# aymenboudhina/Multimodal_VQVAE_compression_audio_tactile

Hardware: AMD Instinct MI355X
Metric: encode+VQ+decode token-frames/sec (1 frame = 13.33 ms of paired 24 kHz audio+tactile) (higher is better)
Workload: dtype f32

## Files before the change

multimodal_vqvae_compression_audio_tactile_amd/csrc/api.hip:

```cpp
#include <hip/hip_runtime.h>
#include <stdarg.h>
#include <math.h>
#include <stdio.h>
#include <string.h>
#include "../../include/mvq.h"
#include "conv_dispatch.hpp"
#include "kernels_small.hpp"

#include <map>
#include <string>
#include <vector>

namespace mvq {
namespace {
struct ProfRec { std::string name; double flops; hipEvent_t e0, e1; };
std::vector<ProfRec> g_prof;
std::vector<hipEvent_t> g_prof_pool;
bool g_prof_on = false;
hipError_t g_prof_err = hipSuccess;
hipEvent_t prof_event()
{
    if (!g_prof_pool.empty()) { hipEvent_t e = g_prof_pool.back(); g_prof_pool.pop_back(); return e; }
    hipEvent_t e = nullptr;
    const hipError_t rc = hipEventCreate(&e);
    if (rc != hipSuccess) { if (g_prof_err == hipSuccess) g_prof_err = rc; return nullptr; }
    return e;
}
}
bool prof_enabled() { return g_prof_on; }
int prof_begin(const char* kernel_name, double flops, hipStream_t s)
{
    if (!g_prof_on) return -1;
    ProfRec r{kernel_name, flops, prof_event(), nullptr};
    if (!r.e0) return -1;
    r.e1 = prof_event();
    if (!r.e1) { g_prof_pool.push_back(r.e0); return -1; }
    const hipError_t rc = hipEventRecord(r.e0, s);
    if (rc != hipSuccess) {
        if (g_prof_err == hipSuccess) g_prof_err = rc;
        g_prof_pool.push_back(r.e0); g_prof_pool.push_back(r.e1);
        return -1;
    }
    g_prof.push_back(r);
    return (int)g_prof.size() - 1;
}
void prof_end(int idx, hipStream_t s)
{
    if (idx < 0 || idx >= (int)g_prof.size()) return;
    const hipError_t rc = hipEventRecord(g_prof[idx].e1, s);
    if (rc != hipSuccess && g_prof_err == hipSuccess) g_prof_err = rc;
}
}

namespace {
thread_local char g_err[512] = "";

int fail(int code, const char* fmt, ...)
{
    va_list ap; va_start(ap, fmt); vsnprintf(g_err, sizeof(g_err), fmt, ap); va_end(ap);
    return code;
}
int hipfail(hipError_t e, const char* what)
{
    return fail(MVQ_EHIP, "%s: %s", what, hipGetErrorString(e));
}
inline hipStream_t S(void* s) { return reinterpret_cast<hipStream_t>(s); }
}
namespace mvq {
void set_last_error(const char* msg) { snprintf(g_err, sizeof(g_err), "%s", msg); }
}
namespace {
inline int conv_out_len(int tin, int ks, int stride, int dil, int pad)
{
    const int span = tin + 2 * pad - dil * (ks - 1) - 1;
    return span < 0 ? 0 : span / stride + 1;
}
}

extern "C" {

int mvq_profile_begin(void)
{
    for (auto& r : mvq::g_prof) { mvq::g_prof_pool.push_back(r.e0); mvq::g_prof_pool.push_back(r.e1); }
    mvq::g_prof.clear();
    mvq::g_prof_err = hipSuccess;
    mvq::g_prof_on = true;
    return MVQ_OK;
}

// ... 36 lines not shown
    std::map<std::string, mvq_profile_entry> agg;
    for (auto& r : mvq::g_prof) {
        hipError_t e = hipEventSynchronize(r.e1);
        if (e != hipSuccess) { recycle(); return hipfail(e, "profile_end: hipEventSynchronize"); }
        float ms = 0.0f;
        e = hipEventElapsedTime(&ms, r.e0, r.e1);
        if (e != hipSuccess) { recycle(); return hipfail(e, "profile_end: hipEventElapsedTime"); }
        auto it = agg.find(r.name);
        if (it == agg.end()) {
            mvq_profile_entry z{};
            snprintf(z.kernel, sizeof(z.kernel), "%s", r.name.c_str());
            it = agg.emplace(r.name, z).first;
        }
        it->second.seconds += 1e-3 * (double)ms;
        it->second.flops += r.flops;
        it->second.launches += 1;
    }
    recycle();
    int i = 0;
    for (auto& kv : agg) {
        if (i >= max_entries) break;
        out[i++] = kv.second;
    }
    *n_entries = i;
    if (n_total) *n_total = (int)agg.size();
    return MVQ_OK;
}

int mvq_abi_version(void) { return 3; }
unsigned mvq_build_flags(void) { return getenv("MVQ_NO_DMA") ? 0x100u : 0u; }
const char* mvq_last_error(void) { return g_err; }

int mvq_device_query(int* cu_count, int* lds_bytes_per_cu, char* arch, int arch_len)
{
    int dev = 0;
    hipError_t e = hipGetDevice(&dev);
    if (e != hipSuccess) return hipfail(e, "hipGetDevice");
    hipDeviceProp_t p;
    e = hipGetDeviceProperties(&p, dev);
    if (e != hipSuccess) return hipfail(e, "hipGetDeviceProperties");
    if (cu_count) *cu_count = p.multiProcessorCount;
    if (lds_bytes_per_cu) *lds_bytes_per_cu = (int)p.maxSharedMemoryPerMultiProcessor;
    if (arch && arch_len > 0) { strncpy(arch, p.gcnArchName, arch_len - 1); arch[arch_len - 1] = 0; }
    return MVQ_OK;
}

int mvq_weight_norm_f32(const float* v, const float* g, float* w, int rows, int inner, void* stream)
{
    if (!v || !g || !w || rows <= 0 || inner <= 0) return fail(MVQ_EINVAL, "weight_norm: bad argument");
    hipError_t e = mvq::launch_weight_norm(v, g, w, rows, inner, S(stream));
    return e == hipSuccess ? MVQ_OK : hipfail(e, "weight_norm");
}

size_t mvq_conv1d_packed_floats(int cin, int cout, int ks)
{
    if (cin <= 0 || cout <= 0 || ks <= 0) return 0;
    return (size_t)cin * ks * mvq::conv_mpad(cout);
}

int mvq_conv1d_pack_f32(const float* w, float* wp, int cin, int cout, int ks, void* stream)
{
    if (!w || !wp || cin <= 0 || cout <= 0 || ks <= 0) return fail(MVQ_EINVAL, "conv1d_pack: bad argument");
    hipError_t e = mvq::launch_pack_conv1d(w, wp, cin, cout, ks, mvq::conv_mpad(cout), S(stream));
    return e == hipSuccess ? MVQ_OK : hipfail(e, "conv1d_pack");
}

size_t mvq_conv_transpose1d_packed_floats(int cin, int cout, int stride)
{
    if (cin <= 0 || cout <= 0 || stride <= 0) return 0;
    return (size_t)cin * 2 * mvq::conv_mpad(cout * stride);
}

int mvq_conv_transpose1d_pack_f32(const float* w, float* wp, int cin, int cout, int stride, void* stream)
{
    if (!w || !wp || cin <= 0 || cout <= 0 || stride <= 0) return fail(MVQ_EINVAL, "conv_transpose1d_pack: bad argument");
    hipError_t e = mvq::launch_pack_convtr(w, wp, cin, cout, stride, mvq::conv_mpad(cout * stride), S(stream));
    return e == hipSuccess ? MVQ_OK : hipfail(e, "conv_transpose1d_pack");
}

static hipError_t dispatch_conv1d(const mvq::ConvArgs& a, int ks, int stride, int dil, hipStream_t s)
{
    const int bm = mvq::conv_tile_bm(a.Cout);
    hipError_t e = hipErrorInvalidValue;
    if (a.Cout >= 16 && a.Cin >= 32 && mvq::conv_underfilled(a) && mvq::conv_lat_wanted(a, ks)) {
        e = mvq::launch_conv_lat(a, ks, stride, dil, s);
        if (e != hipErrorInvalidValue) return e;
    }
    if (a.Cout >= 32 && a.Cin >= 32) {
        if (ks == 7 && stride == 1 && a.Cin % 8 == 0) e = mvq::launch_conv_k7(a, dil, bm, s);
        else if (ks == 1 && stride == 1 && dil == 1 && a.Cin % 32 == 0) e = mvq::launch_conv_k1k3(a, 1, bm, s);
        else if (ks == 3 && stride == 1 && dil == 1 && a.Cin % 16 == 0) e = mvq::launch_conv_k1k3(a, 3, bm, s);
        else if (ks == 2 * stride && dil == 1 && a.Cin % 16 == 0) e = mvq::launch_conv_strided(a, stride, bm, s);
    }
    return e;
}

static hipError_t dispatch_convtr(const mvq::ConvArgs& a, hipStream_t s)
{
    if (a.Cin % 32 != 0 || a.Mrows < 64) return hipErrorInvalidValue;
    return mvq::launch_conv_tr(a, mvq::conv_tile_bm(a.Mrows), s);
}

size_t mvq_bf16x3_split_bytes(int batch, int c, int t)
{
    if (batch <= 0 || c <= 0 || t <= 0) return 0;
    return (size_t)batch * c * t * 6;
}
int mvq_bf16x3_split_f32(const float* x, void* xs, int batch, int c, int t, void* stream)
{
    if (batch < 0 || c <= 0 || t < 0 || c % 8 != 0) return fail(MVQ_EINVAL, "bf16x3_split: bad shape B=%d C=%d T=%d (C %% 8 == 0)", batch, c, t);
    if (batch == 0 || t == 0) return MVQ_OK;
    if (!x || !xs) return fail(MVQ_EINVAL, "bf16x3_split: null tensor");
    if ((reinterpret_cast<uintptr_t>(xs) & 15) != 0) return fail(MVQ_EINVAL, "bf16x3_split: xs must be 16-byte aligned");
    const hipError_t e = mvq::launch_bf16x3_split(x, xs, batch, c, t, S(stream));
    return e == hipSuccess ? MVQ_OK : hipfail(e, "bf16x3_split");
}
size_t mvq_conv1d_k7_bf16x3_packed_bytes(int cout, int cin)
{
    if (cout <= 0 || cin <= 0 || mvq::bf16x6_tile_rows(cout) == 0 || cin % 16 != 0) return 0;
    return (size_t)cout * cin * 7 * 6;
}
int mvq_conv1d_k7_pack_bf16x3(const float* w, void* wq, int cout, int cin, int dgrad, void* stream)
{
    if (cout <= 0 || cin <= 0 || mvq::bf16x6_tile_rows(cout) == 0 || cin % 16 != 0)
        return fail(MVQ_EINVAL, "conv1d_k7_pack_bf16x3: Cout %d must be a multiple of 128 or 96 and Cin %d of 16", cout, cin);
    if (!w || !wq) return fail(MVQ_EINVAL, "conv1d_k7_pack_bf16x3: null tensor");
    if ((reinterpret_cast<uintptr_t>(wq) & 15) != 0) return fail(MVQ_EINVAL, "conv1d_k7_pack_bf16x3: wq must be 16-byte aligned");
    const hipError_t e = mvq::launch_bf16x3_pack_k7(w, wq, cout, cin, dgrad != 0, S(stream));
    return e == hipSuccess ? MVQ_OK : hipfail(e, "conv1d_k7_pack_bf16x3");
}
int mvq_conv1d_k7_bf16x6_f32(const void* xs, const void* wq, const float* bias, const float* alpha_out, float* y, float* y2,
                             const float* dsn_src, const float* dsn_alpha, const float* residual,
                             int batch, int cin, int t, int cout, int dil, int tvalid, void* stream)
{
    if (batch < 0 || cin <= 0 || cout <= 0 || t < 0 || mvq::bf16x6_tile_rows(cout) == 0 || cin % 16 != 0)
        return fail(MVQ_EINVAL, "conv1d_k7_bf16x6: bad shape B=%d Cin=%d T=%d Cout=%d (Cout %% 128 or 96, Cin %% 16)", batch, cin, t, cout);
    if (dil != 1 && dil != 3 && dil != 9) return fail(MVQ_EINVAL, "conv1d_k7_bf16x6: dilation %d not in {1, 3, 9}", dil);
    if (tvalid < 0 || tvalid > t) return fail(MVQ_EINVAL, "conv1d_k7_bf16x6: tvalid %d outside [0, %d]", tvalid, t);
    if (batch == 0 || t == 0) return MVQ_OK;
    if (!xs || !wq || !y) return fail(MVQ_EINVAL, "conv1d_k7_bf16x6: null tensor");
    if (((reinterpret_cast<uintptr_t>(xs) | reinterpret_cast<uintptr_t>(wq)) & 15) != 0)
        return fail(MVQ_EINVAL, "conv1d_k7_bf16x6: xs / wq must be 16-byte aligned");
    if ((long long)batch * ((t + 127) / 128) > 0x7fffffffLL) return fail(MVQ_EINVAL, "conv1d_k7_bf16x6: grid too large");
    if (y2 && !alpha_out) return fail(MVQ_EINVAL, "conv1d_k7_bf16x6: the dual output needs alpha_out");
    if ((dsn_src != nullptr) != (dsn_alpha != nullptr)) return fail(MVQ_EINVAL, "conv1d_k7_bf16x6: dsn_src and dsn_alpha go together");
    mvq::K7Extra ex; ex.y2 = y2; ex.dsn_src = dsn_src; ex.dsn_alpha = dsn_alpha; ex.residual = residual;
    const hipError_t e = mvq::launch_conv_k7_bf16x6(xs, wq, bias, alpha_out, y, batch, cin, t, cout, dil, tvalid, ex, S(stream));
    return e == hipSuccess ? MVQ_OK : hipfail(e, "conv1d_k7_bf16x6");
}

int mvq_f16x2_split_f32(const float* x, void* xs, uint32_t* xamax, int batch, int c, int t, void* stream)
{
    if (batch < 0 || c <= 0 || t < 0 || c % 8 != 0) return fail(MVQ_EINVAL, "f16x2_split: bad shape B=%d C=%d T=%d (C %% 8 == 0)", batch, c, t);
    if (batch == 0 || t == 0) return MVQ_OK;
    if (!x || !xs || !xamax) return fail(MVQ_EINVAL, "f16x2_split: null tensor");
    if ((reinterpret_cast<uintptr_t>(xs) & 15) != 0) return fail(MVQ_EINVAL, "f16x2_split: xs must be 16-byte aligned");
    const hipError_t e = mvq::launch_f16x2_split(x, xs, xamax, batch, c, t, S(stream));
    return e == hipSuccess ? MVQ_OK : hipfail(e, "f16x2_split");
}
size_t mvq_conv1d_k7_f16x2_packed_bytes(int cout, int cin)
{
    if (cout <= 0 || cin <= 0 || mvq::bf16x6_tile_rows(cout) == 0 || cin % 16 != 0) return 0;
    return (size_t)cout * cin * 7 * 4;
}
int mvq_conv1d_k7_pack_f16x2(const float* w, void* wq, uint32_t* wamax, int cout, int cin, int dgrad, void* stream)
{
    if (cout <= 0 || cin <= 0 || mvq::bf16x6_tile_rows(cout) == 0 || cin % 16 != 0)
// ... 832 lines not shown
```

multimodal_vqvae_compression_audio_tactile_amd/csrc/conv_k1k3.hip:

```cpp
#include "conv_dispatch.hpp"
namespace mvq {
hipError_t launch_conv_k1k3(const ConvArgs& a, int ks, int bm, hipStream_t s)
{
    if (ks == 1) {
        if (bm != 96 && conv_prefer_small_tiles(a)) return launch_conv1d_mfma<1, 1, 1, 32, 1, 1, 2, 2, 0>(a, s);
        if (bm == 128) {
            const int tail = a.name_out ? 0 : conv_tail_width(a);
            if (tail) {
                ConvArgs m = a, t = a;
                m.n_tiles_max = a.Ncols / 128;
                t.n_base = m.n_tiles_max * 128;
                hipError_t e = launch_conv1d_mfma<1, 1, 1, 16, 2, 2, 2, 2, 0>(m, s);
                if (e != hipSuccess) return e;
                return tail == 96 ? launch_conv1d_mfma<1, 1, 1, 16, 1, 3, 4, 1, 0>(t, s)
                                  : launch_conv1d_mfma<1, 1, 1, 16, 2, 1, 2, 2, 0>(t, s);
            }
        }
        switch (bm) {
            case 128: return launch_conv1d_mfma<1, 1, 1, 16, 2, 2, 2, 2, 0>(a, s);
            case 96:
                      return (long)a.B * ((a.Ncols + 127) / 128) * ((a.Mrows + 95) / 96) < 200
                                 ? launch_conv1d_mfma<1, 1, 1, 32, 3, 1, 1, 4, 0>(a, s)
                                 : launch_conv1d_mfma<1, 1, 1, 16, 3, 1, 1, 4, 0>(a, s);
            case 64:  return launch_conv1d_mfma<1, 1, 1, 16, 2, 2, 1, 4, 0>(a, s);
        }
    } else if (ks == 3) {
        if (bm != 96 && conv_prefer_small_tiles(a)) return launch_conv1d_mfma<3, 1, 1, 16, 1, 1, 2, 2, 0>(a, s);
        if (bm == 128 && a.Ncols <= 96) return launch_conv1d_mfma<3, 1, 1, 8, 1, 3, 4, 1, 0>(a, s);
        switch (bm) {
            case 128: return conv_dma_rows_ok(a) ? launch_conv1d_mfma<3, 1, 1, 8, 2, 2, 2, 2, 0>(a, s)
                                                 : launch_conv1d_mfma<3, 1, 1, 16, 2, 2, 2, 2, 0>(a, s);
        }
    }
    return hipErrorInvalidValue;
}
}
```

multimodal_vqvae_compression_audio_tactile_amd/csrc/conv_k7.hip:

```cpp
#include "conv_dispatch.hpp"
namespace mvq {
template <int DIL>
static hipError_t k7(const ConvArgs& a, int bm, hipStream_t s)
{
    if (DIL == 1 && bm == 128 && a.Ncols <= 96 && !conv_prefer_small_tiles(a))
        return launch_conv1d_mfma<7, 1, 1, 4, 1, 3, 4, 1, 0>(a, s);
    if (bm != 96 && conv_prefer_small_tiles(a)) return launch_conv1d_mfma<7, 1, DIL, 8, 1, 1, 2, 2, 0>(a, s);
    if (bm == 128) {
        const int tail = a.name_out ? 0 : conv_tail_width(a);
        if (tail) {
            ConvArgs m = a, t = a;
            m.n_tiles_max = a.Ncols / 128;
            t.n_base = m.n_tiles_max * 128;
            hipError_t e = launch_conv1d_mfma<7, 1, DIL, 4, 2, 2, 2, 2, 0>(m, s);
            if (e != hipSuccess) return e;
            return tail == 96 ? launch_conv1d_mfma<7, 1, DIL, 4, 1, 3, 4, 1, 0>(t, s)
                              : launch_conv1d_mfma<7, 1, DIL, 4, 2, 1, 2, 2, 0>(t, s);
        }
    }
    switch (bm) {
        case 128: return launch_conv1d_mfma<7, 1, DIL, 4, 2, 2, 2, 2, 0>(a, s);
        case 96:  return launch_conv1d_mfma<7, 1, DIL, 4, 3, 1, 1, 4, 0>(a, s);
        case 64:  return launch_conv1d_mfma<7, 1, DIL, 8, 2, 2, 1, 4, 0>(a, s);
    }
    return hipErrorInvalidValue;
}
hipError_t launch_conv_k7(const ConvArgs& a, int dil, int bm, hipStream_t s)
{
    switch (dil) {
        case 1: return k7<1>(a, bm, s);
        case 3: return k7<3>(a, bm, s);
        case 9: return k7<9>(a, bm, s);
    }
    return hipErrorInvalidValue;
}
}
```

multimodal_vqvae_compression_audio_tactile_amd/csrc/conv_strided.hip:

```cpp
#include "conv_dispatch.hpp"
namespace mvq {
hipError_t launch_conv_strided(const ConvArgs& a, int stride, int bm, hipStream_t s)
{
    const bool dma = conv_dma_rows_ok(a);
    if (bm == 96 && stride == 2) return dma ? launch_conv1d_mfma<4, 2, 1, 4, 3, 1, 1, 4, 0>(a, s) : launch_conv1d_mfma<4, 2, 1, 8, 3, 1, 1, 4, 0>(a, s);
    if (bm != 128) return hipErrorInvalidValue;
    if (conv_prefer_small_tiles(a)) {
        switch (stride) {
            case 2: return launch_conv1d_mfma<4, 2, 1, 16, 1, 1, 2, 2, 0>(a, s);
            case 4: return launch_conv1d_mfma<8, 4, 1, 8, 1, 1, 2, 2, 0>(a, s);
            case 5: return launch_conv1d_mfma<10, 5, 1, 4, 1, 1, 2, 2, 0>(a, s);
            case 8: return launch_conv1d_mfma<16, 8, 1, 4, 1, 1, 2, 2, 0>(a, s);
        }
    }
    const int tail = a.name_out ? 0 : conv_tail_width(a);
    if (tail && (stride == 4 || stride == 5)) {
        ConvArgs m = a, t = a;
        m.n_tiles_max = a.Ncols / 128;
        t.n_base = m.n_tiles_max * 128;
        hipError_t e = stride == 4 ? (dma ? launch_conv1d_mfma<8, 4, 1, 2, 2, 2, 2, 2, 0>(m, s) : launch_conv1d_mfma<8, 4, 1, 4, 2, 2, 2, 2, 0>(m, s))
                                   : launch_conv1d_mfma<10, 5, 1, 2, 2, 2, 2, 2, 0>(m, s);
        if (e != hipSuccess) return e;
        if (stride == 4) return tail == 96 ? launch_conv1d_mfma<8, 4, 1, 2, 1, 3, 4, 1, 0>(t, s) : launch_conv1d_mfma<8, 4, 1, 2, 2, 1, 2, 2, 0>(t, s);
        return tail == 96 ? launch_conv1d_mfma<10, 5, 1, 2, 1, 3, 4, 1, 0>(t, s) : launch_conv1d_mfma<10, 5, 1, 2, 2, 1, 2, 2, 0>(t, s);
    }
    switch (stride) {
        case 2: return dma ? launch_conv1d_mfma<4, 2, 1, 4, 2, 2, 2, 2, 0>(a, s) : launch_conv1d_mfma<4, 2, 1, 8, 2, 2, 2, 2, 0>(a, s);
        case 4: return dma ? launch_conv1d_mfma<8, 4, 1, 2, 2, 2, 2, 2, 0>(a, s) : launch_conv1d_mfma<8, 4, 1, 4, 2, 2, 2, 2, 0>(a, s);
        case 5: return launch_conv1d_mfma<10, 5, 1, 2, 2, 2, 2, 2, 0>(a, s);
        case 8: if (a.Ncols <= 96) return dma ? launch_conv1d_mfma<16, 8, 1, 1, 1, 3, 4, 1, 0>(a, s) : launch_conv1d_mfma<16, 8, 1, 2, 1, 3, 4, 1, 0>(a, s);
                return dma ? launch_conv1d_mfma<16, 8, 1, 1, 2, 2, 2, 2, 0>(a, s) : launch_conv1d_mfma<16, 8, 1, 2, 2, 2, 2, 2, 0>(a, s);
    }
    return hipErrorInvalidValue;
}
}
```

multimodal_vqvae_compression_audio_tactile_amd/csrc/conv_tr.hip:

```cpp
#include "conv_dispatch.hpp"
namespace mvq {
hipError_t launch_conv_tr(const ConvArgs& a, int bm, hipStream_t s)
{
    if (bm == 128 && conv_prefer_small_tiles(a)) {
        switch (a.up_s) {
            case 8: return launch_conv1d_mfma<2, 1, 1, 32, 1, 1, 2, 2, 8>(a, s);
            case 5: return launch_conv1d_mfma<2, 1, 1, 32, 1, 1, 2, 2, 5>(a, s);
            case 4: return launch_conv1d_mfma<2, 1, 1, 32, 1, 1, 2, 2, 4>(a, s);
            case 2: return launch_conv1d_mfma<2, 1, 1, 32, 1, 1, 2, 2, 2>(a, s);
        }
    }
    const bool dma = conv_dma_rows_ok(a);
    const int tail = (a.name_out || bm != 128) ? 0 : conv_tail_width(a);
    if (tail && (a.up_s == 4 || a.up_s == 5)) {
        ConvArgs m = a, t = a;
        m.n_tiles_max = a.Ncols / 128;
        t.n_base = m.n_tiles_max * 128;
        hipError_t e;
        if (a.up_s == 4) e = dma ? launch_conv1d_mfma<2, 1, 1, 8, 2, 2, 2, 2, 4>(m, s) : launch_conv1d_mfma<2, 1, 1, 16, 2, 2, 2, 2, 4>(m, s);
        else e = dma ? launch_conv1d_mfma<2, 1, 1, 8, 2, 2, 2, 2, 5>(m, s) : launch_conv1d_mfma<2, 1, 1, 16, 2, 2, 2, 2, 5>(m, s);
        if (e != hipSuccess) return e;
        if (a.up_s == 4) return tail == 96 ? launch_conv1d_mfma<2, 1, 1, 8, 1, 3, 4, 1, 4>(t, s) : launch_conv1d_mfma<2, 1, 1, 8, 2, 1, 2, 2, 4>(t, s);
        return tail == 96 ? launch_conv1d_mfma<2, 1, 1, 8, 1, 3, 4, 1, 5>(t, s) : launch_conv1d_mfma<2, 1, 1, 8, 2, 1, 2, 2, 5>(t, s);
    }
    const bool narrow = bm == 128 && a.Ncols <= 96;
    switch (a.up_s) {
        case 8: if (bm == 128 && narrow) return dma ? launch_conv1d_mfma<2, 1, 1, 8, 1, 3, 4, 1, 8>(a, s) : launch_conv1d_mfma<2, 1, 1, 16, 1, 3, 4, 1, 8>(a, s);
                if (bm == 128) return dma ? launch_conv1d_mfma<2, 1, 1, 8, 2, 2, 2, 2, 8>(a, s) : launch_conv1d_mfma<2, 1, 1, 16, 2, 2, 2, 2, 8>(a, s);
                break;
        case 5: if (bm == 128) return dma ? launch_conv1d_mfma<2, 1, 1, 8, 2, 2, 2, 2, 5>(a, s) : launch_conv1d_mfma<2, 1, 1, 16, 2, 2, 2, 2, 5>(a, s);
                break;
        case 4: if (bm == 128) return dma ? launch_conv1d_mfma<2, 1, 1, 8, 2, 2, 2, 2, 4>(a, s) : launch_conv1d_mfma<2, 1, 1, 16, 2, 2, 2, 2, 4>(a, s);
                break;
        case 2: if (bm == 96) return dma ? launch_conv1d_mfma<2, 1, 1, 8, 3, 1, 1, 4, 2>(a, s) : launch_conv1d_mfma<2, 1, 1, 16, 3, 1, 1, 4, 2>(a, s);
                if (bm == 128) return dma ? launch_conv1d_mfma<2, 1, 1, 8, 2, 2, 2, 2, 2>(a, s) : launch_conv1d_mfma<2, 1, 1, 16, 2, 2, 2, 2, 2>(a, s);
                break;
    }
    return hipErrorInvalidValue;
}
}
```

multimodal_vqvae_compression_audio_tactile_amd/dac.py:

```python
from __future__ import annotations

import math
import os
from typing import List, Optional

import torch
import torch.nn as nn

from . import ops
from ._lib import MvqError

ENC_RATES = (2, 4, 5, 8)
DEC_RATES = (8, 5, 4, 2)

PLAN_ENV = ("MVQ_RU_PRESNAKED", "MVQ_VPACKED_LATENTS", "MVQ_PACKED_MIN_BATCH", "MVQ_PACKED_LATENTS", "MVQ_PY_PLAN")
PLAN_OVERRIDES = {k: os.environ[k] for k in PLAN_ENV if k in os.environ}
HOST_ENV_SEEN = {k: os.environ[k] for k in ("MVQ_TWO_STREAM_MAX_BATCH", "MVQ_AR_FUSED_MAX_BATCH", "MVQ_AR_STAGED_MAX_BATCH") if k in os.environ}
USE_STACKS = not PLAN_OVERRIDES


def plan_overrides():
    return sorted(PLAN_OVERRIDES) + sorted(HOST_ENV_SEEN)


class _Packed:

    def __init__(self):
        self._key = None
        self.value = None

    def invalidate(self):
        self._key = None

    def get(self, params, make):
        key = tuple((id(p), p._version, p.data_ptr(), str(p.device)) for p in params)
        if key != self._key:
            self.value = make()
            self._key = key
        return self.value


def _stack_of(mod, describe):
    st = getattr(mod, "_stack_state", None)
    if st is None or st.get("probe") is None:
        probe = describe()
        named = dict(mod.named_parameters())
        st = mod._stack_state = {"probe": probe, "params": [named[n] for n in probe.param_names()], "stamp": None, "stack": None}
    ps = st["params"]
    stamp = (sum(p._version for p in ps), ps[0].data_ptr(), ps[-1].data_ptr(), ps[0].device)
    if stamp != st["stamp"]:
        st["stack"] = st["probe"].bind(ps)
        st["stamp"] = stamp
    return st["stack"]


class Snake1d(nn.Module):

    def __init__(self, channels: int):
        super().__init__()
        self.alpha = nn.Parameter(torch.ones(1, channels, 1))

    def flat(self) -> torch.Tensor:
        return self.alpha.detach().reshape(-1).float().contiguous()


class _WNKeys:

    def _load_from_state_dict(self, state_dict, prefix, *args, **kwargs):
        for new, old in (("parametrizations.weight.original0", "weight_g"), ("parametrizations.weight.original1", "weight_v")):
            if prefix + new in state_dict and prefix + old not in state_dict:
                state_dict[prefix + old] = state_dict.pop(prefix + new)
        super()._load_from_state_dict(state_dict, prefix, *args, **kwargs)


class WNConv1d(_WNKeys, nn.Module):

    def __init__(self, cin, cout, kernel_size, stride=1, dilation=1, padding=0):
        super().__init__()
        self.cin, self.cout, self.ks = cin, cout, kernel_size
        self.stride, self.dilation, self.padding = stride, dilation, padding
        v = torch.randn(cout, cin, kernel_size) / math.sqrt(cin * kernel_size)
        self.weight_g = nn.Parameter(v.reshape(cout, -1).norm(dim=1).reshape(cout, 1, 1))
        self.weight_v = nn.Parameter(v)
        self.bias = nn.Parameter(torch.zeros(cout))
        self._packed = _Packed()

    def packed(self) -> torch.Tensor:
        return self._packed.get((self.weight_g, self.weight_v),
                                lambda: ops.pack_conv1d(ops.weight_norm(self.weight_v.detach(), self.weight_g.detach())))

    def folded_weight(self) -> torch.Tensor:
        return ops.weight_norm(self.weight_v.detach(), self.weight_g.detach())

    def packed_bf16x3(self) -> torch.Tensor:
        if not hasattr(self, "_packed_bf"):
            self._packed_bf = _Packed()
        return self._packed_bf.get((self.weight_g, self.weight_v), lambda: ops.pack_conv1d_k7_bf16x3(self.folded_weight()))

    def packed_f16x2(self):
        if not hasattr(self, "_packed_f16"):
# ... 520 lines not shown
```

Measured before the change: 60700.

## Add analytic cost model to pick conv MFMA tile shape per launch

Introduces a per-family tile cost model using measured efficiency tables, CU wave quantization and LDS-limited residency. Each conv launcher (k1, k3, k7, strided, transposed) builds candidate tiles and keeps the current choice unless another is predicted cheaper by a margin. An MVQ_CONV_TILE env override is also added for forcing a tile. The aim is to reduce wave-quantization and underfill losses on small grids; the risk is model error picking a slower tile, plus getenv overhead on every launch.

After: 60650 (median of 2 runs). Within noise of the previous version (-0.1%).

```diff
diff --git a/multimodal_vqvae_compression_audio_tactile_amd/csrc/api.hip b/multimodal_vqvae_compression_audio_tactile_amd/csrc/api.hip
--- a/multimodal_vqvae_compression_audio_tactile_amd/csrc/api.hip
+++ b/multimodal_vqvae_compression_audio_tactile_amd/csrc/api.hip
@@ -5,6 +5,7 @@
 #include <string.h>
 #include "../../include/mvq.h"
 #include "conv_dispatch.hpp"
+#include "conv_tile_model.hpp"
 #include "kernels_small.hpp"
 
 #include <map>
@@ -207,7 +208,8 @@
 {
     const int bm = mvq::conv_tile_bm(a.Cout);
     hipError_t e = hipErrorInvalidValue;
-    if (a.Cout >= 16 && a.Cin >= 32 && mvq::conv_underfilled(a) && mvq::conv_lat_wanted(a, ks)) {
+    if (a.Cout >= 16 && a.Cin >= 32 && mvq::conv_underfilled(a) && mvq::conv_lat_wanted(a, ks) &&
+        mvq::conv_tile_forced() == mvq::TILE_NONE) {
         e = mvq::launch_conv_lat(a, ks, stride, dil, s);
         if (e != hipErrorInvalidValue) return e;
     }
diff --git a/multimodal_vqvae_compression_audio_tactile_amd/csrc/conv_k1k3.hip b/multimodal_vqvae_compression_audio_tactile_amd/csrc/conv_k1k3.hip
--- a/multimodal_vqvae_compression_audio_tactile_amd/csrc/conv_k1k3.hip
+++ b/multimodal_vqvae_compression_audio_tactile_amd/csrc/conv_k1k3.hip
@@ -1,10 +1,19 @@
 #include "conv_dispatch.hpp"
+#include "conv_tile_model.hpp"
 namespace mvq {
 hipError_t launch_conv_k1k3(const ConvArgs& a, int ks, int bm, hipStream_t s)
 {
     if (ks == 1) {
-        if (bm != 96 && conv_prefer_small_tiles(a)) return launch_conv1d_mfma<1, 1, 1, 32, 1, 1, 2, 2, 0>(a, s);
         if (bm == 128) {
+            const TileCand c[5] = {tile_cand<1, 1, 1, 16, 2, 2, 2, 2, 0>(TILE_128x128, a), tile_cand<1, 1, 1, 16, 1, 3, 4, 1, 0>(TILE_128x96, a),
+                                   tile_cand<1, 1, 1, 16, 2, 1, 2, 2, 0>(TILE_128x64, a), tile_cand<1, 1, 1, 16, 1, 2, 2, 2, 0>(TILE_64x128, a),
+                                   tile_cand<1, 1, 1, 32, 1, 1, 2, 2, 0>(TILE_64x64, a)};
+            switch (conv_choose_tile(a, FAM_K1, a.Cin, 1, c, 5, conv_prefer_small_tiles(a) ? TILE_64x64 : TILE_128x128)) {
+                case TILE_128x96: return launch_conv1d_mfma<1, 1, 1, 16, 1, 3, 4, 1, 0>(a, s);
+                case TILE_128x64: return launch_conv1d_mfma<1, 1, 1, 16, 2, 1, 2, 2, 0>(a, s);
+                case TILE_64x128: return launch_conv1d_mfma<1, 1, 1, 16, 1, 2, 2, 2, 0>(a, s);
+                case TILE_64x64:  return launch_conv1d_mfma<1, 1, 1, 32, 1, 1, 2, 2, 0>(a, s);
+            }
             const int tail = a.name_out ? 0 : conv_tail_width(a);
             if (tail) {
                 ConvArgs m = a, t = a;
@@ -15,22 +24,32 @@
                 return tail == 96 ? launch_conv1d_mfma<1, 1, 1, 16, 1, 3, 4, 1, 0>(t, s)
                                   : launch_conv1d_mfma<1, 1, 1, 16, 2, 1, 2, 2, 0>(t, s);
             }
+            return launch_conv1d_mfma<1, 1, 1, 16, 2, 2, 2, 2, 0>(a, s);
         }
         switch (bm) {
-            case 128: return launch_conv1d_mfma<1, 1, 1, 16, 2, 2, 2, 2, 0>(a, s);
             case 96:
                       return (long)a.B * ((a.Ncols + 127) / 128) * ((a.Mrows + 95) / 96) < 200
                                  ? launch_conv1d_mfma<1, 1, 1, 32, 3, 1, 1, 4, 0>(a, s)
                                  : launch_conv1d_mfma<1, 1, 1, 16, 3, 1, 1, 4, 0>(a, s);
-            case 64:  return launch_conv1d_mfma<1, 1, 1, 16, 2, 2, 1, 4, 0>(a, s);
+            case 64: {
+                const TileCand c[2] = {tile_cand<1, 1, 1, 16, 2, 2, 1, 4, 0>(TILE_64x256, a), tile_cand<1, 1, 1, 32, 1, 1, 2, 2, 0>(TILE_64x64, a)};
+                return conv_choose_tile(a, FAM_K1, a.Cin, 1, c, 2, conv_prefer_small_tiles(a) ? TILE_64x64 : TILE_64x256) == TILE_64x64
+                           ? launch_conv1d_mfma<1, 1, 1, 32, 1, 1, 2, 2, 0>(a, s) : launch_conv1d_mfma<1, 1, 1, 16, 2, 2, 1, 4, 0>(a, s);
+            }
         }
     } else if (ks == 3) {
-        if (bm != 96 && conv_prefer_small_tiles(a)) return launch_conv1d_mfma<3, 1, 1, 16, 1, 1, 2, 2, 0>(a, s);
-        if (bm == 128 && a.Ncols <= 96) return launch_conv1d_mfma<3, 1, 1, 8, 1, 3, 4, 1, 0>(a, s);
-        switch (bm) {
-            case 128: return conv_dma_rows_ok(a) ? launch_conv1d_mfma<3, 1, 1, 8, 2, 2, 2, 2, 0>(a, s)
-                                                 : launch_conv1d_mfma<3, 1, 1, 16, 2, 2, 2, 2, 0>(a, s);
+        if (bm != 128) {
+            if (bm != 96 && conv_prefer_small_tiles(a)) return launch_conv1d_mfma<3, 1, 1, 16, 1, 1, 2, 2, 0>(a, s);
+            return hipErrorInvalidValue;
         }
+        const bool dma = conv_dma_rows_ok(a);
+        const TileCand c[3] = {dma ? tile_cand<3, 1, 1, 8, 2, 2, 2, 2, 0>(TILE_128x128, a) : tile_cand<3, 1, 1, 16, 2, 2, 2, 2, 0>(TILE_128x128, a),
+                               tile_cand<3, 1, 1, 8, 1, 3, 4, 1, 0>(TILE_128x96, a), tile_cand<3, 1, 1, 16, 1, 1, 2, 2, 0>(TILE_64x64, a)};
+        switch (conv_choose_tile(a, FAM_K3, a.Cin * 3, 3, c, 3, conv_prefer_small_tiles(a) ? TILE_64x64 : (a.Ncols <= 96 ? TILE_128x96 : TILE_128x128))) {
+            case TILE_64x64:  return launch_conv1d_mfma<3, 1, 1, 16, 1, 1, 2, 2, 0>(a, s);
+            case TILE_128x96: return launch_conv1d_mfma<3, 1, 1, 8, 1, 3, 4, 1, 0>(a, s);
+        }
+        return dma ? launch_conv1d_mfma<3, 1, 1, 8, 2, 2, 2, 2, 0>(a, s) : launch_conv1d_mfma<3, 1, 1, 16, 2, 2, 2, 2, 0>(a, s);
     }
     return hipErrorInvalidValue;
 }
diff --git a/multimodal_vqvae_compression_audio_tactile_amd/csrc/conv_k7.hip b/multimodal_vqvae_compression_audio_tactile_amd/csrc/conv_k7.hip
--- a/multimodal_vqvae_compression_audio_tactile_amd/csrc/conv_k7.hip
+++ b/multimodal_vqvae_compression_audio_tactile_amd/csrc/conv_k7.hip
@@ -1,29 +1,37 @@
 #include "conv_dispatch.hpp"
+#include "conv_tile_model.hpp"
 namespace mvq {
 template <int DIL>
 static hipError_t k7(const ConvArgs& a, int bm, hipStream_t s)
 {
-    if (DIL == 1 && bm == 128 && a.Ncols <= 96 && !conv_prefer_small_tiles(a))
-        return launch_conv1d_mfma<7, 1, 1, 4, 1, 3, 4, 1, 0>(a, s);
-    if (bm != 96 && conv_prefer_small_tiles(a)) return launch_conv1d_mfma<7, 1, DIL, 8, 1, 1, 2, 2, 0>(a, s);
-    if (bm == 128) {
-        const int tail = a.name_out ? 0 : conv_tail_width(a);
-        if (tail) {
-            ConvArgs m = a, t = a;
-            m.n_tiles_max = a.Ncols / 128;
-            t.n_base = m.n_tiles_max * 128;
-            hipError_t e = launch_conv1d_mfma<7, 1, DIL, 4, 2, 2, 2, 2, 0>(m, s);
-            if (e != hipSuccess) return e;
-            return tail == 96 ? launch_conv1d_mfma<7, 1, DIL, 4, 1, 3, 4, 1, 0>(t, s)
-                              : launch_conv1d_mfma<7, 1, DIL, 4, 2, 1, 2, 2, 0>(t, s);
-        }
+    if (bm == 96) return launch_conv1d_mfma<7, 1, DIL, 4, 3, 1, 1, 4, 0>(a, s);
+    if (bm == 64) {
+        const TileCand c[2] = {tile_cand<7, 1, DIL, 8, 2, 2, 1, 4, 0>(TILE_64x256, a), tile_cand<7, 1, DIL, 8, 1, 1, 2, 2, 0>(TILE_64x64, a)};
+        const int t = conv_choose_tile(a, DIL == 9 ? FAM_K7D9 : FAM_K7, a.Cin * 7, 7, c, 2, conv_prefer_small_tiles(a) ? TILE_64x64 : TILE_64x256);
+        return t == TILE_64x64 ? launch_conv1d_mfma<7, 1, DIL, 8, 1, 1, 2, 2, 0>(a, s) : launch_conv1d_mfma<7, 1, DIL, 8, 2, 2, 1, 4, 0>(a, s);
     }
-    switch (bm) {
-        case 128: return launch_conv1d_mfma<7, 1, DIL, 4, 2, 2, 2, 2, 0>(a, s);
-        case 96:  return launch_conv1d_mfma<7, 1, DIL, 4, 3, 1, 1, 4, 0>(a, s);
-        case 64:  return launch_conv1d_mfma<7, 1, DIL, 8, 2, 2, 1, 4, 0>(a, s);
+    if (bm != 128) return hipErrorInvalidValue;
+    const int today = conv_prefer_small_tiles(a) ? TILE_64x64 : ((DIL == 1 && a.Ncols <= 96) ? TILE_128x96 : TILE_128x128);
+    const TileCand c[5] = {tile_cand<7, 1, DIL, 4, 2, 2, 2, 2, 0>(TILE_128x128, a), tile_cand<7, 1, DIL, 4, 1, 3, 4, 1, 0>(TILE_128x96, a),
+                           tile_cand<7, 1, DIL, 4, 2, 1, 2, 2, 0>(TILE_128x64, a), tile_cand<7, 1, DIL, 4, 1, 2, 2, 2, 0>(TILE_64x128, a),
+                           tile_cand<7, 1, DIL, 8, 1, 1, 2, 2, 0>(TILE_64x64, a)};
+    switch (conv_choose_tile(a, DIL == 9 ? FAM_K7D9 : FAM_K7, a.Cin * 7, 7, c, 5, today)) {
+        case TILE_128x96: return launch_conv1d_mfma<7, 1, DIL, 4, 1, 3, 4, 1, 0>(a, s);
+        case TILE_128x64: return launch_conv1d_mfma<7, 1, DIL, 4, 2, 1, 2, 2, 0>(a, s);
+        case TILE_64x128: return launch_conv1d_mfma<7, 1, DIL, 4, 1, 2, 2, 2, 0>(a, s);
+        case TILE_64x64:  return launch_conv1d_mfma<7, 1, DIL, 8, 1, 1, 2, 2, 0>(a, s);
     }
-    return hipErrorInvalidValue;
+    const int tail = a.name_out ? 0 : conv_tail_width(a);
+    if (tail) {
+        ConvArgs m = a, t = a;
+        m.n_tiles_max = a.Ncols / 128;
+        t.n_base = m.n_tiles_max * 128;
+        hipError_t e = launch_conv1d_mfma<7, 1, DIL, 4, 2, 2, 2, 2, 0>(m, s);
+        if (e != hipSuccess) return e;
+        return tail == 96 ? launch_conv1d_mfma<7, 1, DIL, 4, 1, 3, 4, 1, 0>(t, s)
+                          : launch_conv1d_mfma<7, 1, DIL, 4, 2, 1, 2, 2, 0>(t, s);
+    }
+    return launch_conv1d_mfma<7, 1, DIL, 4, 2, 2, 2, 2, 0>(a, s);
 }
 hipError_t launch_conv_k7(const ConvArgs& a, int dil, int bm, hipStream_t s)
 {
diff --git a/multimodal_vqvae_compression_audio_tactile_amd/csrc/conv_strided.hip b/multimodal_vqvae_compression_audio_tactile_amd/csrc/conv_strided.hip
--- a/multimodal_vqvae_compression_audio_tactile_amd/csrc/conv_strided.hip
+++ b/multimodal_vqvae_compression_audio_tactile_amd/csrc/conv_strided.hip
@@ -1,16 +1,57 @@
 #include "conv_dispatch.hpp"
+#include "conv_tile_model.hpp"
 namespace mvq {
 hipError_t launch_conv_strided(const ConvArgs& a, int stride, int bm, hipStream_t s)
 {
     const bool dma = conv_dma_rows_ok(a);
     if (bm == 96 && stride == 2) return dma ? launch_conv1d_mfma<4, 2, 1, 4, 3, 1, 1, 4, 0>(a, s) : launch_conv1d_mfma<4, 2, 1, 8, 3, 1, 1, 4, 0>(a, s);
     if (bm != 128) return hipErrorInvalidValue;
-    if (conv_prefer_small_tiles(a)) {
+    {
+        const int ktot = a.Cin * 2 * stride;
+        const int today = conv_prefer_small_tiles(a) ? TILE_64x64 : ((stride == 8 && a.Ncols <= 96) ? TILE_128x96 : TILE_128x128);
+        TileCand c[4];
+        int n = 0;
         switch (stride) {
-            case 2: return launch_conv1d_mfma<4, 2, 1, 16, 1, 1, 2, 2, 0>(a, s);
-            case 4: return launch_conv1d_mfma<8, 4, 1, 8, 1, 1, 2, 2, 0>(a, s);
-            case 5: return launch_conv1d_mfma<10, 5, 1, 4, 1, 1, 2, 2, 0>(a, s);
-            case 8: return launch_conv1d_mfma<16, 8, 1, 4, 1, 1, 2, 2, 0>(a, s);
+            case 2: c[n++] = dma ? tile_cand<4, 2, 1, 4, 2, 2, 2, 2, 0>(TILE_128x128, a) : tile_cand<4, 2, 1, 8, 2, 2, 2, 2, 0>(TILE_128x128, a);
+                    c[n++] = tile_cand<4, 2, 1, 16, 1, 1, 2, 2, 0>(TILE_64x64, a);
+                    break;
+            case 4: c[n++] = dma ? tile_cand<8, 4, 1, 2, 2, 2, 2, 2, 0>(TILE_128x128, a) : tile_cand<8, 4, 1, 4, 2, 2, 2, 2, 0>(TILE_128x128, a);
+                    c[n++] = tile_cand<8, 4, 1, 2, 1, 3, 4, 1, 0>(TILE_128x96, a);
+                    c[n++] = tile_cand<8, 4, 1, 2, 2, 1, 2, 2, 0>(TILE_128x64, a);
+                    c[n++] = tile_cand<8, 4, 1, 8, 1, 1, 2, 2, 0>(TILE_64x64, a);
+                    break;
+            case 5: c[n++] = tile_cand<10, 5, 1, 2, 2, 2, 2, 2, 0>(TILE_128x128, a);
+                    c[n++] = tile_cand<10, 5, 1, 2, 1, 3, 4, 1, 0>(TILE_128x96, a);
+                    c[n++] = tile_cand<10, 5, 1, 2, 2, 1, 2, 2, 0>(TILE_128x64, a);
+                    c[n++] = tile_cand<10, 5, 1, 4, 1, 1, 2, 2, 0>(TILE_64x64, a);
+                    break;
+            case 8: c[n++] = dma ? tile_cand<16, 8, 1, 1, 2, 2, 2, 2, 0>(TILE_128x128, a) : tile_cand<16, 8, 1, 2, 2, 2, 2, 2, 0>(TILE_128x128, a);
+                    c[n++] = dma ? tile_cand<16, 8, 1, 1, 1, 3, 4, 1, 0>(TILE_128x96, a) : tile_cand<16, 8, 1, 2, 1, 3, 4, 1, 0>(TILE_128x96, a);
+                    c[n++] = tile_cand<16, 8, 1, 4, 1, 1, 2, 2, 0>(TILE_64x64, a);
+                    break;
+            default: return hipErrorInvalidValue;
+        }
+        const int t = conv_choose_tile(a, stride == 2 ? FAM_S2 : stride == 4 ? FAM_S4 : stride == 5 ? FAM_S5 : FAM_S8, ktot, 2 * stride, c, n, today);
+        if (t == TILE_64x64) {
+            switch (stride) {
+                case 2: return launch_conv1d_mfma<4, 2, 1, 16, 1, 1, 2, 2, 0>(a, s);
+                case 4: return launch_conv1d_mfma<8, 4, 1, 8, 1, 1, 2, 2, 0>(a, s);
+                case 5: return launch_conv1d_mfma<10, 5, 1, 4, 1, 1, 2, 2, 0>(a, s);
+                case 8: return launch_conv1d_mfma<16, 8, 1, 4, 1, 1, 2, 2, 0>(a, s);
+            }
+        }
+        if (t == TILE_128x96) {
+            switch (stride) {
+                case 4: return launch_conv1d_mfma<8, 4, 1, 2, 1, 3, 4, 1, 0>(a, s);
+                case 5: return launch_conv1d_mfma<10, 5, 1, 2, 1, 3, 4, 1, 0>(a, s);
+                case 8: return dma ? launch_conv1d_mfma<16, 8, 1, 1, 1, 3, 4, 1, 0>(a, s) : launch_conv1d_mfma<16, 8, 1, 2, 1, 3, 4, 1, 0>(a, s);
+            }
+        }
+        if (t == TILE_128x64) {
+            switch (stride) {
+                case 4: return launch_conv1d_mfma<8, 4, 1, 2, 2, 1, 2, 2, 0>(a, s);
+                case 5: return launch_conv1d_mfma<10, 5, 1, 2, 2, 1, 2, 2, 0>(a, s);
+            }
         }
     }
     const int tail = a.name_out ? 0 : conv_tail_width(a);
@@ -28,8 +69,7 @@
         case 2: return dma ? launch_conv1d_mfma<4, 2, 1, 4, 2, 2, 2, 2, 0>(a, s) : launch_conv1d_mfma<4, 2, 1, 8, 2, 2, 2, 2, 0>(a, s);
         case 4: return dma ? launch_conv1d_mfma<8, 4, 1, 2, 2, 2, 2, 2, 0>(a, s) : launch_conv1d_mfma<8, 4, 1, 4, 2, 2, 2, 2, 0>(a, s);
         case 5: return launch_conv1d_mfma<10, 5, 1, 2, 2, 2, 2, 2, 0>(a, s);
-        case 8: if (a.Ncols <= 96) return dma ? launch_conv1d_mfma<16, 8, 1, 1, 1, 3, 4, 1, 0>(a, s) : launch_conv1d_mfma<16, 8, 1, 2, 1, 3, 4, 1, 0>(a, s);
-                return dma ? launch_conv1d_mfma<16, 8, 1, 1, 2, 2, 2, 2, 0>(a, s) : launch_conv1d_mfma<16, 8, 1, 2, 2, 2, 2, 2, 0>(a, s);
+        case 8: return dma ? launch_conv1d_mfma<16, 8, 1, 1, 2, 2, 2, 2, 0>(a, s) : launch_conv1d_mfma<16, 8, 1, 2, 2, 2, 2, 2, 0>(a, s);
     }
     return hipErrorInvalidValue;
 }
diff --git a/multimodal_vqvae_compression_audio_tactile_amd/csrc/conv_tile_model.hpp b/multimodal_vqvae_compression_audio_tactile_amd/csrc/conv_tile_model.hpp
--- /dev/null
+++ b/multimodal_vqvae_compression_audio_tactile_amd/csrc/conv_tile_model.hpp
@@ -0,0 +1,108 @@
+#pragma once
+#include <cstdlib>
+#include <cstring>
+#include "conv1d_mfma.hpp"
+
+namespace mvq {
+
+enum ConvTileId : int { TILE_NONE = -1, TILE_128x128 = 0, TILE_128x96, TILE_128x64, TILE_96x128, TILE_64x256, TILE_64x128, TILE_64x64, TILE_COUNT };
+enum ConvFamily : int { FAM_K7 = 0, FAM_K7D9, FAM_K1, FAM_K3, FAM_S2, FAM_S4, FAM_S5, FAM_S8, FAM_TR2, FAM_TR4, FAM_TR5, FAM_TR8, FAM_COUNT };
+
+struct TileCand { int id, bm, bn, lds_bytes, wpe; };
+
+template <int KS, int STRIDE, int DIL, int CK, int MT, int NT, int WAVES_M, int WAVES_N, int UPS>
+inline TileCand tile_cand(int id, const ConvArgs& a)
+{
+    using C = ConvCfg<KS, STRIDE, DIL, CK, MT, NT, WAVES_M, WAVES_N, UPS>;
+    const bool dma = conv_dma_rows_ok(a) && (size_t)C::LDS_FLOATS_DMA * 4 <= 64 * 1024;
+    const size_t lds = (dma ? (size_t)C::LDS_FLOATS_DMA * 4 : (size_t)C::LDS_FLOATS * 4 + (a.alpha_in ? (size_t)2 * a.Cin * 4 : 0)) + (size_t)3 * C::BM * 4;
+    return TileCand{id, C::BM, C::BN, (int)lds, C::MIN_WPE};
+}
+
+constexpr double TILE_CU_PEAK_FLOP_PER_US = 157.3e6 / 256.0;
+constexpr double TILE_MODEL_MARGIN = 0.95;
+constexpr double TILE_GEN_EXPOSED = 0.3;
+constexpr int TILE_MODEL_MAX_BIG = 600;
+struct TileRate { double rate[3]; double fixed_us; };
+#define TILE_NA {{0.0, 0.0, 0.0}, 0.0}
+constexpr TileRate TILE_RATES[FAM_COUNT][TILE_COUNT] = {
+     {{{0.877, 0.916, 0.924}, 11.3}, {{0.859, 0.903, 0.911},  9.4}, {{0.818, 0.872, 0.888},  8.8}, TILE_NA, TILE_NA, {{0.834, 0.884, 0.902},  7.8}, {{0.813, 0.872, 0.890},  7.7}},
+     {{{0.876, 0.918, 0.926}, 10.9}, {{0.854, 0.896, 0.908},  9.0}, {{0.807, 0.857, 0.881},  8.0}, TILE_NA, TILE_NA, {{0.838, 0.889, 0.905},  8.0}, {{0.807, 0.872, 0.639},  4.6}},
+     {{{0.805, 0.888, 0.896}, 12.5}, {{0.795, 0.858, 0.862},  9.7}, {{0.713, 0.855, 0.854},  9.4}, TILE_NA, TILE_NA, {{0.742, 0.861, 0.859},  8.8}, {{0.715, 0.832, 0.842},  7.4}},
+     {{{0.856, 0.903, 0.915}, 10.6}, {{0.850, 0.888, 0.892},  9.7}, TILE_NA, TILE_NA, TILE_NA, TILE_NA, {{0.786, 0.860, 0.878},  7.4}},
+     {{{0.861, 0.886, 0.893}, 12.9}, TILE_NA, TILE_NA, TILE_NA, TILE_NA, TILE_NA, {{0.678, 0.762, 0.790},  7.2}},
+     {{{0.832, 0.882, 0.894}, 10.6}, {{0.790, 0.865, 0.870},  9.9}, {{0.757, 0.819, 0.842},  7.8}, TILE_NA, TILE_NA, TILE_NA, {{0.668, 0.763, 0.778},  6.9}},
+     {{{0.850, 0.893, 0.898}, 10.2}, {{0.816, 0.883, 0.886},  9.5}, {{0.771, 0.839, 0.854},  8.5}, TILE_NA, TILE_NA, TILE_NA, {{0.789, 0.853, 0.864},  7.6}},
+     {{{0.830, 0.878, 0.883},  6.3}, {{0.762, 0.839, 0.848},  6.2}, TILE_NA, TILE_NA, TILE_NA, TILE_NA, {{0.616, 0.701, 0.734},  6.7}},
+     {{{0.833, 0.886, 0.895}, 19.1}, TILE_NA, TILE_NA, TILE_NA, TILE_NA, TILE_NA, {{0.675, 0.784, 0.801},  9.9}},
+     {{{0.846, 0.898, 0.897}, 18.8}, {{0.833, 0.890, 0.870}, 15.1}, {{0.737, 0.847, 0.847}, 13.2}, TILE_NA, TILE_NA, TILE_NA, {{0.682, 0.772, 0.794},  9.6}},
+     {{{1.304, 1.201, 0.963}, 90.5}, {{1.479, 1.145, 1.085}, 63.1}, {{1.250, 1.078, 0.983}, 45.2}, TILE_NA, TILE_NA, TILE_NA, {{1.078, 1.008, 1.009}, 29.5}},
+     {{{0.852, 0.895, 0.898}, 19.0}, {{0.821, 0.885, 0.870}, 14.1}, TILE_NA, TILE_NA, TILE_NA, TILE_NA, {{0.688, 0.769, 0.799},  9.2}},
+};
+#undef TILE_NA
+
+inline const char* tile_name(int id)
+{
+    static const char* const n[TILE_COUNT] = {"128x128", "128x96", "128x64", "96x128", "64x256", "64x128", "64x64"};
+    return id >= 0 && id < TILE_COUNT ? n[id] : "?";
+}
+
+inline int conv_tile_forced()
+{
+    const char* e = getenv("MVQ_CONV_TILE");
+    if (!e || !*e) return TILE_NONE;
+    for (int i = 0; i < TILE_COUNT; ++i)
+        if (strcmp(e, tile_name(i)) == 0) return i;
+    return TILE_NONE;
+}
+
+inline long tile_blocks_per_cu(const ConvArgs& a, const TileCand& c, int ks)
+{
+    const long cols = a.Ncols - a.n_base;
+    const long rows = (a.Mrows + c.bm - 1) / c.bm;
+    long gx = (long)a.B * ((cols + c.bn - 1) / c.bn);
+    if (rows > 1 && (size_t)a.Cin * ks * a.Mpad * sizeof(float) <= ((size_t)5 << 19)) gx = (gx + 7) / 8 * 8;
+    return (gx * rows + 255) / 256;
+}
+
+inline double tile_time_us(const ConvArgs& a, int fam, const TileCand& c, int ktot, int ks)
+{
+    const long q = tile_blocks_per_cu(a, c, ks);
+    const int granule = (c.lds_bytes + 1279) / 1280 * 1280;
+    int R = (160 * 1024) / granule;
+    if (R > c.wpe) R = c.wpe;
+    if (R > 3) R = 3;
+    if (R < 1) R = 1;
+    const TileRate& r = TILE_RATES[fam][c.id];
+    const double t1 = 2.0 * c.bm * c.bn * (double)ktot / TILE_CU_PEAK_FLOP_PER_US;
+    if (q <= 3) return q * t1 / r.rate[q - 1] + r.fixed_us;
+    const long gens = (q + R - 1) / R;
+    return q * t1 / r.rate[R - 1] + r.fixed_us * (1.0 + TILE_GEN_EXPOSED * (double)(gens - 1));
+}
+
+inline int conv_choose_tile(const ConvArgs& a, int fam, int ktot, int ks, const TileCand* cands, int n, int today)
+{
+    if (a.vp_seg) return today;
+    const int forced = conv_tile_forced();
+    if (forced != TILE_NONE)
+        for (int i = 0; i < n; ++i)
+            if (cands[i].id == forced) return forced;
+    if ((long)a.B * ((a.Ncols + 127) / 128) * ((a.Mrows + 127) / 128) >= TILE_MODEL_MAX_BIG) return today;
+    double t_today = -1.0;
+    for (int i = 0; i < n; ++i)
+        if (cands[i].id == today && TILE_RATES[fam][today].rate[0] > 0.0) {
+            if (tile_blocks_per_cu(a, cands[i], ks) <= 1) return today;
+            t_today = tile_time_us(a, fam, cands[i], ktot, ks);
+        }
+    if (t_today < 0.0 || TILE_RATES[fam][today].rate[0] <= 0.0) return today;
+    int best = today;
+    double t_best = t_today * TILE_MODEL_MARGIN;
+    for (int i = 0; i < n; ++i) {
+        if (cands[i].id == today || TILE_RATES[fam][cands[i].id].rate[0] <= 0.0) continue;
+        const double t = tile_time_us(a, fam, cands[i], ktot, ks);
+        if (t < t_best) { t_best = t; best = cands[i].id; }
+    }
+    return best;
+}
+
+}
diff --git a/multimodal_vqvae_compression_audio_tactile_amd/csrc/conv_tr.hip b/multimodal_vqvae_compression_audio_tactile_amd/csrc/conv_tr.hip
--- a/multimodal_vqvae_compression_audio_tactile_amd/csrc/conv_tr.hip
+++ b/multimodal_vqvae_compression_audio_tactile_amd/csrc/conv_tr.hip
@@ -1,16 +1,53 @@
 #include "conv_dispatch.hpp"
+#include "conv_tile_model.hpp"
 namespace mvq {
 hipError_t launch_conv_tr(const ConvArgs& a, int bm, hipStream_t s)
 {
-    if (bm == 128 && conv_prefer_small_tiles(a)) {
+    const bool dma = conv_dma_rows_ok(a);
+    if (bm == 128) {
+        const int today = conv_prefer_small_tiles(a) ? TILE_64x64 : ((a.up_s == 8 && a.Ncols <= 96) ? TILE_128x96 : TILE_128x128);
+        TileCand c[4];
+        int n = 0;
+#define MVQ_TR_CANDS(U)                                                                                                                  \
+        c[n++] = dma ? tile_cand<2, 1, 1, 8, 2, 2, 2, 2, U>(TILE_128x128, a) : tile_cand<2, 1, 1, 16, 2, 2, 2, 2, U>(TILE_128x128, a);   \
+        c[n++] = tile_cand<2, 1, 1, 32, 1, 1, 2, 2, U>(TILE_64x64, a)
         switch (a.up_s) {
-            case 8: return launch_conv1d_mfma<2, 1, 1, 32, 1, 1, 2, 2, 8>(a, s);
-            case 5: return launch_conv1d_mfma<2, 1, 1, 32, 1, 1, 2, 2, 5>(a, s);
-            case 4: return launch_conv1d_mfma<2, 1, 1, 32, 1, 1, 2, 2, 4>(a, s);
-            case 2: return launch_conv1d_mfma<2, 1, 1, 32, 1, 1, 2, 2, 2>(a, s);
+            case 8: MVQ_TR_CANDS(8);
+                    c[n++] = dma ? tile_cand<2, 1, 1, 8, 1, 3, 4, 1, 8>(TILE_128x96, a) : tile_cand<2, 1, 1, 16, 1, 3, 4, 1, 8>(TILE_128x96, a);
+                    break;
+            case 5: MVQ_TR_CANDS(5);
+                    c[n++] = tile_cand<2, 1, 1, 8, 1, 3, 4, 1, 5>(TILE_128x96, a); c[n++] = tile_cand<2, 1, 1, 8, 2, 1, 2, 2, 5>(TILE_128x64, a);
+                    break;
+            case 4: MVQ_TR_CANDS(4);
+                    c[n++] = tile_cand<2, 1, 1, 8, 1, 3, 4, 1, 4>(TILE_128x96, a); c[n++] = tile_cand<2, 1, 1, 8, 2, 1, 2, 2, 4>(TILE_128x64, a);
+                    break;
+            case 2: MVQ_TR_CANDS(2); break;
+            default: return hipErrorInvalidValue;
+        }
+#undef MVQ_TR_CANDS
+        const int t = conv_choose_tile(a, a.up_s == 2 ? FAM_TR2 : a.up_s == 4 ? FAM_TR4 : a.up_s == 5 ? FAM_TR5 : FAM_TR8, a.Cin * 2, 2, c, n, today);
+        if (t == TILE_64x64) {
+            switch (a.up_s) {
+                case 8: return launch_conv1d_mfma<2, 1, 1, 32, 1, 1, 2, 2, 8>(a, s);
+                case 5: return launch_conv1d_mfma<2, 1, 1, 32, 1, 1, 2, 2, 5>(a, s);
+                case 4: return launch_conv1d_mfma<2, 1, 1, 32, 1, 1, 2, 2, 4>(a, s);
+                case 2: return launch_conv1d_mfma<2, 1, 1, 32, 1, 1, 2, 2, 2>(a, s);
+            }
+        }
+        if (t == TILE_128x96) {
+            switch (a.up_s) {
+                case 8: return dma ? launch_conv1d_mfma<2, 1, 1, 8, 1, 3, 4, 1, 8>(a, s) : launch_conv1d_mfma<2, 1, 1, 16, 1, 3, 4, 1, 8>(a, s);
+                case 5: return launch_conv1d_mfma<2, 1, 1, 8, 1, 3, 4, 1, 5>(a, s);
+                case 4: return launch_conv1d_mfma<2, 1, 1, 8, 1, 3, 4, 1, 4>(a, s);
+            }
+        }
+        if (t == TILE_128x64) {
+            switch (a.up_s) {
+                case 5: return launch_conv1d_mfma<2, 1, 1, 8, 2, 1, 2, 2, 5>(a, s);
+                case 4: return launch_conv1d_mfma<2, 1, 1, 8, 2, 1, 2, 2, 4>(a, s);
+            }
         }
     }
-    const bool dma = conv_dma_rows_ok(a);
     const int tail = (a.name_out || bm != 128) ? 0 : conv_tail_width(a);
     if (tail && (a.up_s == 4 || a.up_s == 5)) {
         ConvArgs m = a, t = a;
@@ -23,10 +60,8 @@
         if (a.up_s == 4) return tail == 96 ? launch_conv1d_mfma<2, 1, 1, 8, 1, 3, 4, 1, 4>(t, s) : launch_conv1d_mfma<2, 1, 1, 8, 2, 1, 2, 2, 4>(t, s);
         return tail == 96 ? launch_conv1d_mfma<2, 1, 1, 8, 1, 3, 4, 1, 5>(t, s) : launch_conv1d_mfma<2, 1, 1, 8, 2, 1, 2, 2, 5>(t, s);
     }
-    const bool narrow = bm == 128 && a.Ncols <= 96;
     switch (a.up_s) {
-        case 8: if (bm == 128 && narrow) return dma ? launch_conv1d_mfma<2, 1, 1, 8, 1, 3, 4, 1, 8>(a, s) : launch_conv1d_mfma<2, 1, 1, 16, 1, 3, 4, 1, 8>(a, s);
-                if (bm == 128) return dma ? launch_conv1d_mfma<2, 1, 1, 8, 2, 2, 2, 2, 8>(a, s) : launch_conv1d_mfma<2, 1, 1, 16, 2, 2, 2, 2, 8>(a, s);
+        case 8: if (bm == 128) return dma ? launch_conv1d_mfma<2, 1, 1, 8, 2, 2, 2, 2, 8>(a, s) : launch_conv1d_mfma<2, 1, 1, 16, 2, 2, 2, 2, 8>(a, s);
                 break;
         case 5: if (bm == 128) return dma ? launch_conv1d_mfma<2, 1, 1, 8, 2, 2, 2, 2, 5>(a, s) : launch_conv1d_mfma<2, 1, 1, 16, 2, 2, 2, 2, 5>(a, s);
                 break;
diff --git a/multimodal_vqvae_compression_audio_tactile_amd/dac.py b/multimodal_vqvae_compression_audio_tactile_amd/dac.py
--- a/multimodal_vqvae_compression_audio_tactile_amd/dac.py
+++ b/multimodal_vqvae_compression_audio_tactile_amd/dac.py
@@ -15,7 +15,7 @@
 
 PLAN_ENV = ("MVQ_RU_PRESNAKED", "MVQ_VPACKED_LATENTS", "MVQ_PACKED_MIN_BATCH", "MVQ_PACKED_LATENTS", "MVQ_PY_PLAN")
 PLAN_OVERRIDES = {k: os.environ[k] for k in PLAN_ENV if k in os.environ}
-HOST_ENV_SEEN = {k: os.environ[k] for k in ("MVQ_TWO_STREAM_MAX_BATCH", "MVQ_AR_FUSED_MAX_BATCH", "MVQ_AR_STAGED_MAX_BATCH") if k in os.environ}
+HOST_ENV_SEEN = {k: os.environ[k] for k in ("MVQ_TWO_STREAM_MAX_BATCH", "MVQ_AR_FUSED_MAX_BATCH", "MVQ_AR_STAGED_MAX_BATCH", "MVQ_CONV_TILE") if k in os.environ}
 USE_STACKS = not PLAN_OVERRIDES
 
 
```
